# arotem3/CuDDHelmholtz

Hardware: AMD Instinct MI355X
Metric: DDH-GMRES DoF*iter/s (higher is better)
Workload: dtype f32

## Files before the change

### cuddhelmholtz_amd/_native.py

```python
from __future__ import annotations

import ctypes as C
import re
from pathlib import Path

ROOT = Path(__file__).resolve().parent.parent
LIB_PATH = Path(__file__).resolve().parent / "lib" / "libcuddh_amd.so"
HEADERS = [ROOT / "include" / "cuddh_hip.h", ROOT / "include" / "cuddh_capi.h"]


class NativeLibraryMissing(RuntimeError):
    pass


def declared_symbols() -> list[str]:
    names: list[str] = []
    for h in HEADERS:
        text = re.sub(r"/\*.*?\*/", "", h.read_text(), flags=re.S)
        for m in re.finditer(r"\b(cuddh_[a-z0-9_]+)\s*\(", text):
            n = m.group(1)
            if n not in names and n != "cuddh_action_cb":
                names.append(n)
    return names

# ... 138 lines not shown
_sig("cuddh_hip_operator_plan_apply", ci, vp, cd, ci, vp, vp, vp)
_sig("cuddh_hip_ddh_geom_setup_f32", ci, ci, ci, ci, ci, vp, vp, vp, vp, vp, vp)
_sig("cuddh_hip_ddh_geom_setup_f64", ci, ci, ci, ci, ci, vp, vp, vp, vp, vp, vp)
_sig("cuddh_hip_ddh_geom_from_corners_f32", ci, ci, ci, vp, vp, vp, vp, vp, vp, vp)
_sig("cuddh_hip_ddh_geom_from_corners_f64", ci, ci, ci, vp, vp, vp, vp, vp, vp, vp)
_sig("cuddh_hip_ddh_plan_create", ci, C.POINTER(vp), C.POINTER(DdhDesc), ci, ci)
_sig("cuddh_hip_ddh_plan_create_general", ci, C.POINTER(vp), C.POINTER(DdhDesc), ci, ci, ci)
_sig("cuddh_hip_ddh_plan_destroy", ci, vp)
_sig("cuddh_hip_ddh_plan_kernel", ci, vp)
_sig("cuddh_hip_ddh_plan_set_wh_iters", ci, vp, ci)
_sig("cuddh_hip_ddh_plan_set_wave_priority", ci, vp, ci)
_sig("cuddh_hip_ddh_plan_set_sweep_form", ci, vp, ci)
_sig("cuddh_hip_ddh_plan_sweep_form", ci, vp)
_sig("cuddh_hip_ddh_plan_set_chain_order", ci, vp, ci)
_sig("cuddh_hip_ddh_plan_chain_order", ci, vp)
_sig("cuddh_hip_ddh_plan_set_owner_rule", ci, vp, ci)
_sig("cuddh_element_lane_tables", ci, ci, vp, vp, vp)
_sig("cuddh_ddh_resolve", ci, *([ci] * 13), vp)
_sig("cuddh_hip_ddh_plan_set_time_grids", ci, vp, ci, vp, vp, vp, vp, vp, vp)
_sig("cuddh_hip_ddh_plan_time_grids", ci, vp)
_sig("cuddh_hip_ddh_plan_set_integrator", ci, vp, ci)
_sig("cuddh_hip_ddh_plan_integrator", ci, vp)
_sig("cuddh_hip_ddh_apply_list_f32", ci, vp, vp, ci, vp, vp, ci, vp, vp, vp)
_sig("cuddh_hip_ddh_apply_list_f64", ci, vp, vp, ci, vp, vp, ci, vp, vp, vp)
_sig("cuddh_hip_ddh_plan_set_vector_layout", ci, vp, vp, ci)
_sig("cuddh_hip_ddh_apply_f32", ci, vp, ci, ci, vp, vp, ci, vp, vp, vp)
_sig("cuddh_hip_ddh_apply_f64", ci, vp, ci, ci, vp, vp, ci, vp, vp, vp)
_sig("cuddh_hip_wave_stage_begin_f64", ci, ci, cd, vp, vp, vp, vp, vp, vp, vp)
_sig("cuddh_hip_wave_stage_rk2_a_f64", ci, ci, cd, cd, cd, *([vp] * 10))
_sig("cuddh_hip_wave_stage_rk2_b_f64", ci, ci, cd, cd, cd, cd, *([vp] * 11))
for _n in ("1", "2", "3"):
    _sig(f"cuddh_hip_wave_stage_rk4_{_n}_f64", ci, ci, cd, cd, cd, *([vp] * 12))
_sig("cuddh_hip_wave_stage_rk4_4_f64", ci, ci, cd, cd, cd, cd, *([vp] * 13))
# ... 103 lines not shown
_sig("cuddh_ddh_create_labels", vp, cd, vp, vp, ci, vp, ci, ci)
_sig("cuddh_ddh_create_labels_integrator", vp, cd, vp, vp, ci, vp, ci, ci, ci, vp, ci, ci, ci)
_sig("cuddh_ddh_create_timegrid", vp, cd, vp, vp, ci, ci, ci, ci, ci, ci, vp, ci)
_sig("cuddh_ddh_time_ratios", ci, vp, vp)
_sig("cuddh_ddh_create_integrator", vp, cd, vp, vp, ci, ci, ci, ci, ci, ci, vp, ci, ci, ci)
_sig("cuddh_ddh_integrator", ci, vp, vp, vp)
_sig("cuddh_ddh_destroy", None, vp)
_sig("cuddh_ddh_size", ci, vp)
_sig("cuddh_ddh_info", ci, vp, vp, vp)
_sig("cuddh_ddh_set_wh_iters", ci, vp, ci)
_sig("cuddh_ddh_set_wave_priority", ci, vp, ci)
_sig("cuddh_ddh_set_sweep_form", ci, vp, ci)
_sig("cuddh_ddh_sweep_form", ci, vp)
_sig("cuddh_ddh_set_chain_order", ci, vp, ci)
_sig("cuddh_ddh_chain_order", ci, vp)
_sig("cuddh_ddh_set_owner_rule", ci, vp, ci)


class MultiGpuResult(C.Structure):
    _fields_ = [("success", ci), ("num_iter", ci), ("num_matvec", ci), ("n_res", ci), ("world", ci), ("used_rccl", ci),
                ("t_setup", cd), ("t_rhs", cd), ("t_gmres", cd), ("t_postprocess", cd), ("bytes_sent_per_action_rank0", C.c_longlong)]


class HelmholtzMultiGpuResult(C.Structure):
    _fields_ = [("success", ci), ("num_iter", ci), ("num_matvec", ci), ("n_res", ci), ("world", ci), ("used_rccl", ci),
                ("t_setup", cd), ("t_apply", cd), ("t_gmres", cd), ("n_loc_max", C.c_longlong), ("n_halo_max", C.c_longlong),
                ("halo_bytes_per_apply_max", C.c_longlong)]


_sig("cuddh_helmholtz_multi_gpu", ci, vp, ci, cd, vp, vp, vp, vp, ci, ci, ci, ci, ci, cd, C.POINTER(HelmholtzMultiGpuResult), vp)
# ... 62 lines not shown
```

### cuddhelmholtz_amd/api.py

```python
from __future__ import annotations

import ctypes as C
from dataclasses import dataclass, field

import numpy as np

from . import _native as N

lib = N.lib


def _ptr(t, dtype=None, numel=None, what="tensor"):
    if t is None:
        return None
    if not t.is_cuda:
        raise ValueError(f"{what}: expected a CUDA tensor")
    if not t.is_contiguous():
        raise ValueError(f"{what}: expected a contiguous tensor")
    if dtype is not None:
        import torch

        want = {"f64": torch.float64, "f32": torch.float32, "i32": torch.int32}.get(dtype, dtype)
        if t.dtype != want:
            raise ValueError(f"{what}: expected dtype {want}, got {t.dtype}")
# ... 504 lines not shown
    def sweep_form(self) -> int:
        form = lib.cuddh_ddh_sweep_form(self._h)
        if form < 0:
            N.check_capi(form, "DDH.sweep_form")
        return form

    def set_chain_order(self, order: int = 0):
        N.check_capi(lib.cuddh_ddh_set_chain_order(self._h, int(order)), "DDH.set_chain_order")

    def chain_order(self) -> int:
        order = lib.cuddh_ddh_chain_order(self._h)
        if order < 0:
            N.check_capi(order, "DDH.chain_order")
        return order

    def set_owner_rule(self, last: bool):
        N.check_capi(lib.cuddh_ddh_set_owner_rule(self._h, 1 if last else 0), "DDH.set_owner_rule")

    def set_wave_priority(self, high: bool):
        N.check_capi(lib.cuddh_ddh_set_wave_priority(self._h, 1 if high else 0), "DDH.set_wave_priority")

    def table(self, name: str) -> np.ndarray:
        n = lib.cuddh_ddh_table(self._h, name.encode(), None, 1)
        if n < 0:
            raise RuntimeError(N.last_error())
        dtype = np.int32 if name in self._INT_TABLES else (np.float64 if self.f64 else np.float32)
        out = np.empty(int(n), dtype=dtype)
        if n:
            lib.cuddh_ddh_table(self._h, name.encode(), _h(out), 0)
        return out
# ... 288 lines not shown
```

### cuddhelmholtz_amd/csrc/include/cuddh/ddh.hpp

```cpp
#ifndef CUDDH_AMD_DDH_HPP
#define CUDDH_AMD_DDH_HPP

#include <memory>
#include <vector>

#include "blas1.hpp"
#include "ensemble.hpp"
#include "krylov.hpp"
#include "memory.hpp"
#include "operator.hpp"
#include "operators.hpp"

struct cuddh_ddh_plan;

namespace cuddh
{
    struct from_labels_t
    {
        explicit constexpr from_labels_t() = default;
    };
    inline constexpr from_labels_t from_labels{};

    struct DDHTimeStep
    {
// ... 47 lines not shown
            int num_domains() const { return n_domains; }
            int num_steps() const { return nt; }
            double time_step() const { return dt; }
            int mesh_steps() const;
            DDHIntegrator integrator() const;
            const std::vector<int> &time_ratios() const;
            const std::vector<int> &time_grid_ratios() const;
            long long time_grid_table(int ratio, int which, const Real *&table) const;
            int kernel_kind() const;
            void set_waveholtz_iterations(int n) const;
            void set_wave_priority(bool high) const;
            void set_sweep_form(int form) const;
            int sweep_form() const;
            void set_chain_order(int order) const;
            int chain_order() const;
            void set_last_copy_publishes(bool last) const;
            const EnsembleSpace &ensemble() const { return *efem; }

            void solve(int dom_begin, int dom_end, const double *x, double *y, bool zero_y, const Real *lambda,
                       Real *update) const;
            void solve_listed(const int *d_domains, int n, const double *x, const Real *lambda, Real *update) const;
            void solve_listed(const int *d_domains, int n, const double *x, double *y, bool zero_y, const Real *lambda, Real *update) const;

            const host_device_ivec &table_B() const { return _Bf; }
            const host_device_ivec &table_gI() const { return _gI; }
            const host_device_ivec &table_sI() const { return _sI; }
            const HostDeviceArray<Real> &table_D() const { return _D; }
            const HostDeviceArray<Real> &table_G() const
            {
                ensure_plan();
// ... 103 lines not shown
```

### cuddhelmholtz_amd/csrc/kernels/ddh.hip

```cpp
#include <algorithm>
#include <cmath>
#include <type_traits>
#include <vector>

#include "ddh_device.hpp"
#include "ddh_element_lane.hpp"
#include "ddh_resolve.hpp"
#include "element_lane_tables.hpp"

using namespace cuddh_k;

struct cuddh_ddh_plan;

namespace
{
    template <typename Real>
    using DdhRun = void (*)(const cuddh_ddh_plan *, const DdhArgs<Real> &, int n_local, hipStream_t);
    struct DdhLaunch
    {
        DdhRun<float> run32 = nullptr;
        DdhRun<double> run64 = nullptr;
        int per_group = 4;
        unsigned block = 256;
        size_t lds = 0;
// ... 7 lines not shown
    DdhResolved now{0, 0, 0};
    DdhLaunch launch;
    unsigned facts = 0;
    int mx_elems = 0;
    int nodes;
    int wh_iters = 5;
    const int *gI_override = nullptr;
    int g_ndof_override = 0;
    float *Aop = nullptr;
    double *Aop64 = nullptr;
    float *Sep = nullptr;
    float *Sep4 = nullptr;
    int last_copy = 0;
    int sweep_form = 0;
    int chain_order = 0;
    int wave_priority = 0;
    int *csr_off = nullptr, *csr_src = nullptr;
    int requested = 0;
    int n_grids = 0;
    void *grids = nullptr;
    const int *grid_of = nullptr;
    const void *grid_filter = nullptr, *grid_cs = nullptr, *grid_sn = nullptr;
    int *by_steps = nullptr;
    int *by_index = nullptr;
    int rk4 = 0;
};

namespace
{
    constexpr int WH_ITERS_REFERENCE = 5;
// ... 1456 lines not shown
                                        { hipLaunchKernelGGL((ddh_wave8_kernel<Real, ASM, SEP>), launch_grid(p, n_local), dim3(p->launch.block), 0, st, A,
                                                             static_cast<const Real *>(p->d.D), fl, cs, sn, reinterpret_cast<const Real *>(p->Sep)); });
    }

    template <typename Real, bool GRIDS, bool RK4>
    void run_mfma(const cuddh_ddh_plan *p, const DdhArgs<Real> &A, int n_local, hipStream_t st)
    {
        const Real *K = sizeof(Real) == 4 ? reinterpret_cast<const Real *>(p->Aop) : reinterpret_cast<const Real *>(p->Aop64);
        with_tables<Real, GRIDS, RK4>(p, [&](const Real *fl, const Real *cs, const Real *sn, auto... o)
                                      { with_flags([&](auto FORCED, auto HOLD)
                                                   { hipLaunchKernelGGL((ddh_mfma_kernel<Real, FORCED.value, HOLD.value, decltype(o)...>), launch_grid(p, n_local),
                                                                        dim3(p->launch.block), 0, st, A, K, fl, cs, sn, o...); },
                                                   A.x != nullptr, A.prio != 0); });
    }

    template <int NB, bool LAST_COPY, bool PAIRED, bool GRIDS>
    void run_element_lane(const cuddh_ddh_plan *p, const DdhArgs<float> &A, int n_local, hipStream_t st)
    {
        with_tables<float, GRIDS, false>(p, [&](const float *fl, const float *cs, const float *sn, auto... o)
                                         { with_flags([&](auto FORCED, auto HOLD)
                                                      { hipLaunchKernelGGL((ddh_element_lane_kernel<NB, FORCED.value, HOLD.value, LAST_COPY, PAIRED, decltype(o)...>),
                                                                           launch_grid(p, n_local), dim3(p->launch.block), 0, st, A, p->Sep4, fl, cs, sn, o...); },
                                                      A.x != nullptr, A.prio != 0); });
    }

    template <bool LAST_COPY, bool GRIDS>
    void run_element_lane8(const cuddh_ddh_plan *p, const DdhArgs<float> &A, int n_local, hipStream_t st)
    {
        with_tables<float, GRIDS, false>(p, [&](const float *fl, const float *cs, const float *sn, auto... o)
                                         { with_flags([&](auto FORCED, auto HOLD)
                                                      { hipLaunchKernelGGL((ddh_element_lane8_kernel<FORCED.value, HOLD.value, LAST_COPY, decltype(o)...>),
                                                                           launch_grid(p, n_local), dim3(p->launch.block), 0, st, A, p->Sep4, fl, cs, sn, o...); },
                                                      A.x != nullptr, A.prio != 0); });
    }

    template <typename Real, bool GRIDS, bool RK4>
    void set_launch(const cuddh_ddh_plan *p, const DdhResolved &r, DdhLaunch &L)
    {
        constexpr bool f32 = sizeof(Real) == 4, plain = !GRIDS && !RK4;
        DdhRun<Real> run = nullptr;
        const bool last_copy = p->last_copy != 0;
        switch (r.kernel)
        {
        case 1:
        case 10:
            L.per_group = 1;
            L.block = p->nodes;
            L.lds = (size_t)p->nodes * (4 * sizeof(Real) + 5 * sizeof(int));
            with_n_basis(p->d.nb, [&](auto NB)
                         {
                             if (p->nodes <= 256)
                                 run = r.kernel == 10 ? run_block<Real, NB.value, true, 256, GRIDS, RK4> : run_block<Real, NB.value, false, 256, GRIDS, RK4>;
// ... 6 lines not shown
            if constexpr (!RK4)
                run = run_wave<Real, f32 ? 1 : 0, GRIDS, RK4>;
            break;
        case 4:
            if constexpr (!RK4)
                run = run_wave<Real, f32 ? 2 : 0, GRIDS, RK4>;
            break;
        case 5:
            if constexpr (f32)
            {
                if (r.form < 2)
                    run = run_mfma<float, GRIDS, RK4>;
                else if constexpr (plain)
                {
                    L.per_group = 16;
                    with_flags([&](auto LAST_COPY, auto PAIRED) { run = run_element_lane<4, LAST_COPY.value, PAIRED.value, false>; }, r.form == 3, r.order == 2);
                }
            }
            break;
        case 8:
            if constexpr (!f32)
                run = run_mfma<double, GRIDS, RK4>;
            break;
        case 6:
        case 7:
            if constexpr (plain)
            {
                L.per_group = 8;
                if constexpr (f32)
                    run = r.kernel == 7 ? run_wave8<float, true, true> : run_wave8<float, true, false>;
                else if (r.kernel == 6)
                    run = run_wave8<double, false, false>;
            }
            break;
        case 9: run = run_general_wave<Real, f32 ? 1 : 0, GRIDS, RK4>; break;
        case 11:
            if constexpr (f32 && !RK4)
                with_flags([&](auto LAST_COPY) { run = run_element_lane8<LAST_COPY.value, GRIDS>; }, last_copy);
            break;
        case 12:
            if constexpr (f32 && plain)
            {
                L.per_group = 16;
                with_flags([&](auto LAST_COPY) { run = run_element_lane<5, LAST_COPY.value, false, false>; }, last_copy);
            }
            break;
        case 13:
            if constexpr (f32 && !RK4)
            {
                L.per_group = 16;
                with_flags(
                    [&](auto LAST_COPY)
                    {
                        if (p->d.nb == 4)
                            run = run_element_lane<4, LAST_COPY.value, false, GRIDS>;
                        else
                            run = run_element_lane<5, LAST_COPY.value, false, GRIDS>;
                    },
                    last_copy);
            }
            break;
        }
        if constexpr (f32)
            L.run32 = run;
        else
            L.run64 = run;
    }

    int resolve(cuddh_ddh_plan *p, int setting = DDH_SET_NONE)
    {
        const DdhShape shape{p->d.nb, p->d.nel1d, p->d.n_domains, p->is_f64, p->mx_elems};
        DdhResolved r;
        if (ddh_resolve(shape, p->requested, p->facts, p->now.kernel, DdhOptions{p->n_grids > 0, p->rk4, p->sweep_form, p->chain_order}, setting, r))
            return static_cast<int>(hipErrorInvalidValue);
        DdhLaunch L;
        with_flags([&](auto F64, auto GRIDS, auto RK4) { set_launch<std::conditional_t<F64.value, double, float>, GRIDS.value, RK4.value>(p, r, L); },
                   p->is_f64 != 0, p->n_grids > 0, p->rk4 != 0);
        if (!L.run32 && !L.run64)
            return static_cast<int>(hipErrorInvalidValue);
        p->now = r;
        p->launch = L;
        return 0;
    }

    template <class Store>
    int set_and_resolve(cuddh_ddh_plan *p, int setting, Store store)
    {
        const cuddh_ddh_plan before = *p;
        store(*p);
        const int err = resolve(p, setting);
        if (err)
            *p = before;
        return err;
    }

// ... 250 lines not shown
            return static_cast<int>(hipErrorInvalidValue);
        return set_and_resolve(plan, DDH_SET_SWEEP_FORM, [&](cuddh_ddh_plan &p) { p.sweep_form = form; });
    }

    int cuddh_hip_ddh_plan_sweep_form(const cuddh_ddh_plan *plan) { return plan ? plan->now.form : 0; }

    int cuddh_hip_ddh_plan_set_chain_order(cuddh_ddh_plan *plan, int order)
    {
        if (!plan)
            return static_cast<int>(hipErrorInvalidValue);
        return set_and_resolve(plan, DDH_SET_CHAIN_ORDER, [&](cuddh_ddh_plan &p) { p.chain_order = order; });
    }

    int cuddh_hip_ddh_plan_chain_order(const cuddh_ddh_plan *plan) { return plan ? plan->now.order : 0; }

    int cuddh_hip_ddh_plan_set_time_grids(cuddh_ddh_plan *plan, int n_grids, const int *h_nt, const double *h_dt, const void *filter,
                                          const void *cs, const void *sn, const int *d_grid_of)
    {
        if (!plan || n_grids < 1 || !h_nt || !h_dt || !filter || !cs || !sn || !d_grid_of)
            return static_cast<int>(hipErrorInvalidValue);
        const int nd = plan->d.n_domains;
        std::vector<int> filt_off(n_grids), cs_off(n_grids);
        long long fo = 0, co = 0;
        for (int g = 0; g < n_grids; ++g)
        {
            if (h_nt[g] < 1 || !(h_dt[g] > 0.0) || !std::isfinite(h_dt[g]))
                return static_cast<int>(hipErrorInvalidValue);
            filt_off[g] = static_cast<int>(fo);
            cs_off[g] = static_cast<int>(co);
            fo += (long long)h_nt[g] + 1;
// ... 117 lines not shown
```

### cuddhelmholtz_amd/csrc/kernels/ddh_element_lane.hpp

```cpp
#ifndef CUDDH_AMD_DDH_ELEMENT_LANE_HPP
#define CUDDH_AMD_DDH_ELEMENT_LANE_HPP

#include <type_traits>

#include "ddh_device.hpp"

namespace
{
#define CUDDH_EL_ASSEMBLE(NAME, SHL, SHR)                                                                                                  \
    __device__ inline void NAME(float (&hi)[4], float (&lo)[4], float mHi, float mLo)                                                      \
    {                                                                                                                                      \
        float t0, t1, t2, t3;                                                                                                              \
        asm volatile("s_nop 1\n\t"                                                                                                         \
                     "v_mul_f32_dpp %8, %0, %13 " SHR " row_mask:0xf bank_mask:0xf bound_ctrl:1\n\t"                                       \
                     "v_mul_f32_dpp %9, %1, %13 " SHR " row_mask:0xf bank_mask:0xf bound_ctrl:1\n\t"                                       \
                     "v_mul_f32_dpp %10, %2, %13 " SHR " row_mask:0xf bank_mask:0xf bound_ctrl:1\n\t"                                      \
                     "v_mul_f32_dpp %11, %3, %13 " SHR " row_mask:0xf bank_mask:0xf bound_ctrl:1\n\t"                                      \
                     "v_fmac_f32_dpp %0, %4, %12 " SHL " row_mask:0xf bank_mask:0xf bound_ctrl:1\n\t"                                      \
                     "v_fmac_f32_dpp %1, %5, %12 " SHL " row_mask:0xf bank_mask:0xf bound_ctrl:1\n\t"                                      \
                     "v_fmac_f32_dpp %2, %6, %12 " SHL " row_mask:0xf bank_mask:0xf bound_ctrl:1\n\t"                                      \
                     "v_fmac_f32_dpp %3, %7, %12 " SHL " row_mask:0xf bank_mask:0xf bound_ctrl:1\n\t"                                      \
                     "v_add_f32 %4, %4, %8\n\t"                                                                                            \
                     "v_add_f32 %5, %5, %9\n\t"                                                                                            \
                     "v_add_f32 %6, %6, %10\n\t"                                                                                           \
// ... 113 lines not shown
    {
        constexpr int EX = NEL - 1, EY = NEL * (NEL - 1);
        const int k = n % NB, l = n / NB;
        const bool first = !(k == 0 && (tid & EX) > 0) && !(l == 0 && (tid & EY) > 0);
        const bool last = !(k == NB - 1 && (tid & EX) < EX) && !(l == NB - 1 && (tid & EY) < EY);
        return LAST_COPY ? last : first;
    }

    typedef float pair_t __attribute__((ext_vector_type(2)));
    constexpr int el_pair(int k, int l) { return k + 4 * ((l == 1 || l == 2) ? 1 : 0); }
    constexpr int el_half(int l) { return l >= 2 ? 1 : 0; }
    constexpr unsigned ELEMENT_INTERIOR_PAIRS = (1u << 5) | (1u << 6);
    constexpr unsigned ELEMENT_LANE_DM_PAIRS(bool forced) { return forced ? 0x60u : 0x1fu; }
    constexpr unsigned ELEMENT_LANE_PAIRED_DM_PAIRS(bool forced) { return forced ? 0x60u : 0xffu; }

    __device__ inline pair_t pk_fma(pair_t a, pair_t b, pair_t c) { return __builtin_elementwise_fma(a, b, c); }
    __device__ inline pair_t pk_fma(float a, pair_t b, pair_t c) { return __builtin_elementwise_fma(pair_t{a, a}, b, c); }
    template <int HALF>
    __device__ inline void pk_fmac_scalar(pair_t &t, pair_t c, pair_t w)
    {
        if constexpr (HALF == 0)
            asm("v_pk_fma_f32 %0, %1, %2, %0 op_sel_hi:[0,1,1]" : "+v"(t) : "s"(c), "v"(w));
        else
            asm("v_pk_fma_f32 %0, %1, %2, %0 op_sel:[1,0,0] op_sel_hi:[1,1,1]" : "+v"(t) : "s"(c), "v"(w));
    }
    constexpr int bx_slot(int k, int j) { return 3 * k + (j < k ? j : j - 1); }
    template <int HALF>
    __device__ inline void pk_fmac_half(pair_t &t, pair_t c, pair_t w)
    {
        if constexpr (HALF == 0)
// ... 160 lines not shown
                    if (((INTERIOR >> l) & 1u) != 0)
                        dq = LEAN == 2 ? pk_fma(s1, Gf[l], pk_fma(c1, F[l], z[l])) : z[l];
                    else
                        dq = pk_fma(s1, Gf[l], pk_fma(c1, F[l], pk_fma(-Hi[l], qh[l], z[l])));
                    if (((DM >> l) & 1u) != 0)
                        q[l] = pk_fma(dm[l], dq, q[l]);
                    else
                        q[l] = pk_fma(hm[l], 2.0f * dq, q[l]);
                    u[l] = pk_fma(kw, p[l], u[l]);
                    v[l] = pk_fma(kw, q[l], v[l]);
                }
            }
        }
    }


    template <int NB, bool FORCED, bool HOLD, bool LAST_COPY, bool PAIRED, typename... Grids>
    __global__ void __launch_bounds__(256, NB == 4 ? 3 : (FORCED ? 1 : 2))
        ddh_element_lane_kernel(DdhArgs<float> A, const float *__restrict__ Sep, const float *__restrict__ filt, const float *__restrict__ cs,
                                const float *__restrict__ sn, Grids... grids)
    {
        constexpr bool GROUPED = sizeof...(Grids) > 0;
        constexpr int NN = NB * NB;
        constexpr int NS = NB == 4 ? 8 : NN;
        using state_t = std::conditional_t<NB == 4, pair_t, float>;
        static_assert(NB == 4 || NB == 5, "the assembly statements exist for 4 and 5 values a side");
        static_assert(sizeof...(Grids) <= 1 && scheme_of<Grids...> == 0, "one grid, or TimeGrids; no RK4 form");
        static_assert(!(PAIRED && NB != 4), "the paired chains are those of the packed form");
        static_assert(!(PAIRED && sizeof...(Grids) > 0), "the paired chains are built for the one-grid kernel only");
        const int s_first = A.dom_begin + 4 * (blockIdx.x * 4 + (threadIdx.x >> 6));
        if (s_first >= A.dom_end)
            return;
        if constexpr (HOLD)
            __builtin_amdgcn_s_setprio(3);
        [[maybe_unused]] const int w_first = wave_uniform(s_first);
        [[maybe_unused]] int done = 0;
        [[maybe_unused]] GroupedRows rows{};
        [[maybe_unused]] DdhArgs<float> Ap;
        const DdhArgs<float> &Ar = [&]() -> const DdhArgs<float> &
        {
            if constexpr (GROUPED)
                return Ap;
            else
                return A;
// ... 94 lines not shown
                for (int l = 0; l < 5; ++l)
                {
                    z[4 + 5 * l] = hi[l];
                    z[0 + 5 * l] = lo[l];
                }
                float up[5] = {z[20], z[21], z[22], z[23], z[24]}, dn[5] = {z[0], z[1], z[2], z[3], z[4]};
                element_assemble_eta_row5_asm(up, dn);
#pragma unroll
                for (int k = 0; k < 5; ++k)
                {
                    z[k + 20] = up[k];
                    z[k] = dn[k];
                }
            }
        };
        if constexpr (NB == 4)
            wh_march_pairs<FORCED ? 2 : 1, ELEMENT_INTERIOR_PAIRS, PAIRED ? ELEMENT_LANE_PAIRED_DM_PAIRS(FORCED) : ELEMENT_LANE_DM_PAIRS(FORCED)>(
                Ar, tg.nt, tg.dt, tg.filt, tg.cs, tg.sn, invm, Hi, F, Gf, u, v, sweep);
        else
            wh_march<FORCED ? 2 : 1, element_interior_registers(NB)>(Ar, tg.nt, tg.dt, tg.filt, tg.cs, tg.sn, invm, Hi, F, Gf, u, v, sweep);

        if constexpr (GROUPED)
        {
            tid = lane_here();
            asm volatile("" : "+s"(done));
            reread_args(Ap);
        }
        else
        {
            tid = threadIdx.x;
            asm volatile("" : "+v"(tid));
// ... 102 lines not shown
```

### cuddhelmholtz_amd/csrc/kernels/ddh_resolve.hpp

```cpp
#pragma once

namespace cuddh_k
{
    enum DdhCheck
    {
        DDH_STRUCTURE = 1,
        DDH_UNIFORM = 2,
        DDH_INTERIOR = 3,
        DDH_DENSE = 4,
        DDH_SEP8 = 5,
        DDH_LANE = 6
    };
    constexpr unsigned ddh_fact(int check) { return 1u << check; }

    struct DdhShape
    {
        int nb, nel1d, n_domains, is_f64;
        int mx_elems;
    };

    struct DdhOptions
    {
        int time_grids;
        int rk4;
        int sweep_form, chain_order;
    };

    enum DdhSetting
    {
        DDH_SET_NONE = 0,
        DDH_SET_SWEEP_FORM = 1,
        DDH_SET_CHAIN_ORDER = 2,
        DDH_SET_OWNER_RULE = 3
    };

    struct DdhResolved
    {
        int kernel;
        int form;
        int order;
    };

    constexpr int DDH_BLOCK_MAX_NODES = 1024;
    constexpr int DDH_GENERAL_MAX_NODES = 256;

    int ddh_checks(const DdhShape &shape, int request);

    int ddh_resolve(const DdhShape &shape, int request, unsigned facts, int current, const DdhOptions &options, int setting, DdhResolved &out);
}
```

### cuddhelmholtz_amd/csrc/src/capi.cpp

```cpp
#include <algorithm>
#include <cmath>
#include <cstdio>
#include <cstring>
#include <exception>
#include <memory>
#include <stdexcept>
#include <string>
#include <vector>

#include "cuddh.hpp"
#include "cuddh_capi.h"
#include "cuddh_hip.h"

using namespace cuddh;

namespace
{
    thread_local std::string g_error;

    template <typename F>
    int guarded(F &&f)
    {
        try
        {
// ... 1070 lines not shown
                h->f64->internals().set_chain_order(order);
            else
                h->f32->internals().set_chain_order(order);
        });
    }
    int cuddh_ddh_chain_order(void *d)
    {
        int order = 0;
        const int err = guarded([&]
        {
            auto *h = static_cast<DdhHandle *>(d);
            order = h->is64() ? h->f64->internals().chain_order() : h->f32->internals().chain_order();
        });
        return err ? -1 : order;
    }
    int cuddh_ddh_set_owner_rule(void *d, int last)
    {
        return guarded([&]
        {
            auto *h = static_cast<DdhHandle *>(d);
            if (h->is64())
                h->f64->internals().set_last_copy_publishes(last != 0);
            else
                h->f32->internals().set_last_copy_publishes(last != 0);
        });
    }
    int cuddh_ddh_sweep_form(void *d)
    {
        int form = 0;
        const int err = guarded([&]
// ... 392 lines not shown
```

### cuddhelmholtz_amd/csrc/src/ddh.cpp

```cpp
#include "cuddh/ddh.hpp"

#include <algorithm>
#include <atomic>
#include <chrono>
#include <cstdio>
#include <cstdlib>
#include <cmath>
#include <string>
#include <type_traits>
#include <vector>

#include "cuddh/parallel.hpp"
#include "cuddh/time_grid.hpp"
#include "cuddh_hip.h"

namespace cuddh
{
    namespace detail
    {
        namespace
        {
            template <typename Real>
            void geom_setup(int n_domains, int mx_elems, int nb, const int *n_elems, const int *elems, const double *w,
                            const double *points, const double *corners, Real *G)
// ... 653 lines not shown
        template <typename Real>
        void DDHCore<Real>::set_chain_order(int order) const
        {
            ensure_plan();
            check_hip(cuddh_hip_ddh_plan_set_chain_order(plan, order), "DDH chain order");
        }

        template <typename Real>
        int DDHCore<Real>::chain_order() const
        {
            ensure_plan();
            return cuddh_hip_ddh_plan_chain_order(plan);
        }

        template <typename Real>
        void DDHCore<Real>::set_last_copy_publishes(bool last) const
        {
            ensure_plan();
            check_hip(cuddh_hip_ddh_plan_set_owner_rule(plan, last ? 1 : 0), "DDH owner rule");
        }

        template <typename Real>
        void DDHCore<Real>::set_wave_priority(bool high) const
        {
            ensure_plan();
            check_hip(cuddh_hip_ddh_plan_set_wave_priority(plan, high ? 1 : 0), "DDH wave priority");
        }

        template <typename Real>
        void DDHCore<Real>::ensure_assembly() const
// ... 223 lines not shown
```

### cuddhelmholtz_amd/csrc/src/ddh_resolve.cpp

```cpp
#include "ddh_resolve.hpp"

#include "cuddh_hip.h"

namespace cuddh_k
{
    namespace
    {
        constexpr int REFUSED = 1;

        constexpr int ELEMENT_LANE_MIN_DOMAINS = 8192;
        constexpr int ELEMENT_LANE5_MIN_DOMAINS = 64;

        constexpr unsigned S = DDH_STRUCTURE, U = DDH_UNIFORM, I = DDH_INTERIOR;
        constexpr unsigned seq(unsigned a, unsigned b = 0, unsigned c = 0, unsigned d = 0, unsigned e = 0)
        {
            return a | (b << 4) | (c << 8) | (d << 12) | (e << 16);
        }

        struct KernelTraits
        {
            int nb, nel1d;
            int real_bytes;
            unsigned checks;
            bool grids, rk4, owner_rule;
// ... 109 lines not shown
                return REFUSED;
            k = k == 3 ? 2 : 1;
        }
        const bool lane_form = k == 5 && (facts & ddh_fact(DDH_LANE)) && !o.time_grids && !o.rk4;
        if (o.sweep_form >= 2 && !lane_form)
            return REFUSED;
        if (setting == DDH_SET_CHAIN_ORDER && o.chain_order == 2 && !lane_form)
            return REFUSED;
        if (setting == DDH_SET_OWNER_RULE && !KERNELS[k].owner_rule)
            return REFUSED;
        out.kernel = k;
        out.form = k != 5 ? 0 : !lane_form ? 1 : o.sweep_form != 0 ? o.sweep_form : s.n_domains >= ELEMENT_LANE_MIN_DOMAINS ? 2 : 1;
        out.order = out.form < 2 ? 0 : o.chain_order != 0 ? o.chain_order : o.sweep_form == 0 ? 2 : 1;
        return 0;
    }
}

extern "C"
{
    int cuddh_ddh_resolve(int nb, int nel1d, int n_domains, int is_f64, int mx_elems, int request, int facts, int current, int time_grids, int rk4,
                          int sweep_form, int chain_order, int setting, int *out)
    {
        using namespace cuddh_k;
        if (!out)
            return 1;
        const DdhShape s{nb, nel1d, n_domains, is_f64 ? 1 : 0, mx_elems};
        out[3] = ddh_checks(s, request);
        DdhResolved r{0, 0, 0};
        const int err = ddh_resolve(s, request, static_cast<unsigned>(facts), current, DdhOptions{time_grids, rk4, sweep_form, chain_order}, setting, r);
        out[0] = r.kernel;
        out[1] = r.form;
        out[2] = r.order;
        return err;
    }
}
```

### include/cuddh_capi.h

```cpp
#ifndef CUDDH_CAPI_H
#define CUDDH_CAPI_H

#include <stddef.h>

#ifdef __cplusplus
extern "C" {
#endif

const char *cuddh_last_error(void);
void cuddh_set_stream(void *stream);
void *cuddh_get_stream(void);

int cuddh_quadrature(int n, int type, double *h_x, double *h_w);
void *cuddh_basis_create(int n);
void cuddh_basis_destroy(void *basis);
int cuddh_basis_eval(void *basis, int m, const double *h_x, double *h_P);
int cuddh_basis_deriv(void *basis, int m, const double *h_x, double *h_D);

void *cuddh_mesh_uniform_rect(int nx, double ax, double bx, int ny, double ay, double by);
void *cuddh_mesh_from_vertices(int n_pts, const double *h_xy, int n_elem, const int *h_elems);
void *cuddh_mesh_load(const char *dir);
void *cuddh_mesh_refined(void *mesh, int times);
int cuddh_mesh_partition(void *mesh, int n_parts, int *h_labels);
void cuddh_mesh_destroy(void *mesh);
// ... 80 lines not shown
    double t_setup, t_apply, t_gmres;
    long long n_loc_max, n_halo_max, halo_bytes_per_apply_max;
} cuddh_helmholtz_multi_gpu_result;
int cuddh_helmholtz_multi_gpu(void *mesh, int nb, double omega, const double *h_a2x, const double *h_ax, const double *h_x, double *h_y,
                              int world, int transport, int reps, int m, int maxit, double tol, cuddh_helmholtz_multi_gpu_result *out,
                              double *h_res );
int cuddh_helmholtz_partition_query(void *mesh, void *fem, void *fs, int rank, int world, int which, int peer, int *h_out);
int cuddh_trace_exchange_query(const int *h_B, int n_domains, int mx_fdof, int n_lambda, int rank, int world, int which, int peer,
                               int *h_out);
int cuddh_ddh_set_wh_iters(void *ddh, int n);
int cuddh_ddh_set_wave_priority(void *ddh, int high);
int cuddh_ddh_set_sweep_form(void *ddh, int form);
int cuddh_ddh_sweep_form(void *ddh);
int cuddh_ddh_set_chain_order(void *ddh, int order);
int cuddh_ddh_chain_order(void *ddh);
int cuddh_ddh_set_owner_rule(void *ddh, int last);
int cuddh_ddh_rhs(void *ddh, const double *f, void *b);
int cuddh_ddh_postprocess(void *ddh, const void *lambda, const double *f, double *u);
int cuddh_ddh_action(void *ddh, const void *x, void *y);
int cuddh_ddh_local_traces(void *ddh, int d0, int d1, const double *f, const void *lambda, void *update);
int cuddh_ddh_local_traces_listed(void *ddh, const int *d_domains, int n, const double *f, const void *lambda, void *update);
int cuddh_ddh_local_solution_listed(void *ddh, const int *d_domains, int n, const void *lambda, const double *f, double *u, int zero_u);
int cuddh_ddh_local_solution(void *ddh, int d0, int d1, const void *lambda, const double *f, double *u, int zero_u);
long long cuddh_ddh_table(void *ddh, const char *name, void *h_out, int count_only);

typedef struct cuddh_solver_result
{
    int success;
    int num_iter;
    int num_matvec;
// ... 67 lines not shown
```

### include/cuddh_hip.h

```cpp
#ifndef CUDDH_HIP_H
#define CUDDH_HIP_H

#include <stddef.h>

#ifdef __cplusplus
extern "C" {
#endif


int cuddh_hip_malloc_zeroed(void **ptr, size_t bytes);
int cuddh_hip_free(void *ptr);
int cuddh_hip_copy_h2d(void *dst, const void *h_src, size_t bytes);
int cuddh_hip_copy_d2h(void *h_dst, const void *src, size_t bytes);
int cuddh_hip_copy_h2d_on(void *dst, const void *h_src, size_t bytes, void *stream);
int cuddh_hip_copy_d2h_on(void *h_dst, const void *src, size_t bytes, void *stream);
int cuddh_hip_copy_d2d(void *dst, const void *src, size_t bytes, void *stream);
int cuddh_hip_memset_zero(void *ptr, size_t bytes, void *stream);
int cuddh_hip_stream_sync(void *stream);
int cuddh_hip_device_sync(void);
int cuddh_hip_device_count(void);
int cuddh_hip_host_alloc(void **ptr, size_t bytes);
int cuddh_hip_host_free(void *ptr);
int cuddh_hip_copy_d2h_async(void *h_dst, const void *src, size_t bytes, void *stream);
int cuddh_hip_event_create(void **ev);
// ... 141 lines not shown
    const void *sn;
} cuddh_ddh_desc;

typedef struct cuddh_ddh_plan cuddh_ddh_plan;
int cuddh_hip_ddh_plan_create(cuddh_ddh_plan **plan, const cuddh_ddh_desc *desc, int is_f64, int kernel);
int cuddh_hip_ddh_plan_create_general(cuddh_ddh_plan **plan, const cuddh_ddh_desc *desc, int mx_elems, int is_f64, int kernel);
int cuddh_hip_ddh_plan_destroy(cuddh_ddh_plan *plan);
int cuddh_hip_ddh_plan_kernel(const cuddh_ddh_plan *plan);
int cuddh_hip_ddh_plan_set_vector_layout(cuddh_ddh_plan *plan, const int *d_gI, int g_ndof);
int cuddh_hip_ddh_plan_set_wave_priority(cuddh_ddh_plan *plan, int high);
int cuddh_hip_ddh_plan_set_wh_iters(cuddh_ddh_plan *plan, int wh_iters);
int cuddh_hip_ddh_plan_set_sweep_form(cuddh_ddh_plan *plan, int form);
int cuddh_hip_ddh_plan_sweep_form(const cuddh_ddh_plan *plan);
int cuddh_hip_ddh_plan_set_chain_order(cuddh_ddh_plan *plan, int order);
int cuddh_hip_ddh_plan_chain_order(const cuddh_ddh_plan *plan);
int cuddh_hip_ddh_plan_set_owner_rule(cuddh_ddh_plan *plan, int last);
int cuddh_element_lane_tables(int nb, const float *h_D, const float *h_G, float *h_out);
int cuddh_ddh_resolve(int nb, int nel1d, int n_domains, int is_f64, int mx_elems, int request, int facts, int current, int time_grids, int rk4,
                      int sweep_form, int chain_order, int setting, int *out);
int cuddh_hip_ddh_plan_set_time_grids(cuddh_ddh_plan *plan, int n_grids, const int *h_nt, const double *h_dt, const void *filter,
                                      const void *cs, const void *sn, const int *d_grid_of);
int cuddh_hip_ddh_plan_time_grids(const cuddh_ddh_plan *plan);
int cuddh_hip_ddh_plan_set_integrator(cuddh_ddh_plan *plan, int scheme);
int cuddh_hip_ddh_plan_integrator(const cuddh_ddh_plan *plan);

int cuddh_hip_ddh_apply_f32(const cuddh_ddh_plan *plan, int dom_begin, int dom_end, const double *x, double *y,
                            int zero_y, const float *lambda, float *update, void *stream);
int cuddh_hip_ddh_apply_f64(const cuddh_ddh_plan *plan, int dom_begin, int dom_end, const double *x, double *y,
                            int zero_y, const double *lambda, double *update, void *stream);
int cuddh_hip_ddh_apply_list_f32(const cuddh_ddh_plan *plan, const int *d_domains, int n, const double *x, double *y, int zero_y,
                                 const float *lambda, float *update, void *stream);
int cuddh_hip_ddh_apply_list_f64(const cuddh_ddh_plan *plan, const int *d_domains, int n, const double *x, double *y, int zero_y,
                                 const double *lambda, double *update, void *stream);

// ... 106 lines not shown
```

Baseline: 118.1 million.

## Apply wave-march sources only in first WH pass and reuse forced response

Adds a packed wave-march variant for the paired-chain element-lane kernel. The source terms are applied only in the first WaveHoltz pass. That forced response is parked in shared memory and added back after each later pass, which runs source-free, relying on linearity. The variant is selected by a new forcing setting that defaults to on when the chain order resolves to paired. This removes the per-step source FMAs and cos/sin table loads from later passes. In exchange it adds a large shared-memory buffer that may lower occupancy, and it changes the floating-point summation order.

```diff
diff --git a/cuddhelmholtz_amd/_native.py b/cuddhelmholtz_amd/_native.py
--- a/cuddhelmholtz_amd/_native.py
+++ b/cuddhelmholtz_amd/_native.py
@@ -176,9 +176,12 @@
 _sig("cuddh_hip_ddh_plan_sweep_form", ci, vp)
 _sig("cuddh_hip_ddh_plan_set_chain_order", ci, vp, ci)
 _sig("cuddh_hip_ddh_plan_chain_order", ci, vp)
+_sig("cuddh_hip_ddh_plan_set_forcing", ci, vp, ci)
+_sig("cuddh_hip_ddh_plan_forcing", ci, vp)
 _sig("cuddh_hip_ddh_plan_set_owner_rule", ci, vp, ci)
 _sig("cuddh_element_lane_tables", ci, ci, vp, vp, vp)
 _sig("cuddh_ddh_resolve", ci, *([ci] * 13), vp)
+_sig("cuddh_ddh_resolve_forcing", ci, *([ci] * 14), vp)
 _sig("cuddh_hip_ddh_plan_set_time_grids", ci, vp, ci, vp, vp, vp, vp, vp, vp)
 _sig("cuddh_hip_ddh_plan_time_grids", ci, vp)
 _sig("cuddh_hip_ddh_plan_set_integrator", ci, vp, ci)
@@ -312,6 +315,8 @@
 _sig("cuddh_ddh_sweep_form", ci, vp)
 _sig("cuddh_ddh_set_chain_order", ci, vp, ci)
 _sig("cuddh_ddh_chain_order", ci, vp)
+_sig("cuddh_ddh_set_forcing", ci, vp, ci)
+_sig("cuddh_ddh_forcing", ci, vp)
 _sig("cuddh_ddh_set_owner_rule", ci, vp, ci)
 
 
diff --git a/cuddhelmholtz_amd/api.py b/cuddhelmholtz_amd/api.py
--- a/cuddhelmholtz_amd/api.py
+++ b/cuddhelmholtz_amd/api.py
@@ -542,6 +542,15 @@
             N.check_capi(order, "DDH.chain_order")
         return order
 
+    def set_forcing(self, forcing: int = 0):
+        N.check_capi(lib.cuddh_ddh_set_forcing(self._h, int(forcing)), "DDH.set_forcing")
+
+    def forcing(self) -> int:
+        forcing = lib.cuddh_ddh_forcing(self._h)
+        if forcing < 0:
+            N.check_capi(forcing, "DDH.forcing")
+        return forcing
+
     def set_owner_rule(self, last: bool):
         N.check_capi(lib.cuddh_ddh_set_owner_rule(self._h, 1 if last else 0), "DDH.set_owner_rule")
 
diff --git a/cuddhelmholtz_amd/csrc/include/cuddh/ddh.hpp b/cuddhelmholtz_amd/csrc/include/cuddh/ddh.hpp
--- a/cuddhelmholtz_amd/csrc/include/cuddh/ddh.hpp
+++ b/cuddhelmholtz_amd/csrc/include/cuddh/ddh.hpp
@@ -85,6 +85,8 @@
             int sweep_form() const;
             void set_chain_order(int order) const;
             int chain_order() const;
+            void set_forcing(int forcing) const;
+            int forcing() const;
             void set_last_copy_publishes(bool last) const;
             const EnsembleSpace &ensemble() const { return *efem; }
 
diff --git a/cuddhelmholtz_amd/csrc/kernels/ddh.hip b/cuddhelmholtz_amd/csrc/kernels/ddh.hip
--- a/cuddhelmholtz_amd/csrc/kernels/ddh.hip
+++ b/cuddhelmholtz_amd/csrc/kernels/ddh.hip
@@ -45,6 +45,8 @@
     int last_copy = 0;
     int sweep_form = 0;
     int chain_order = 0;
+    int forcing = 0;
+    int forcing_now = 0;
     int wave_priority = 0;
     int *csr_off = nullptr, *csr_src = nullptr;
     int requested = 0;
@@ -1531,12 +1533,12 @@
                                                    A.x != nullptr, A.prio != 0); });
     }
 
-    template <int NB, bool LAST_COPY, bool PAIRED, bool GRIDS>
+    template <int NB, bool LAST_COPY, bool PAIRED, bool ONCE, bool GRIDS>
     void run_element_lane(const cuddh_ddh_plan *p, const DdhArgs<float> &A, int n_local, hipStream_t st)
     {
         with_tables<float, GRIDS, false>(p, [&](const float *fl, const float *cs, const float *sn, auto... o)
                                          { with_flags([&](auto FORCED, auto HOLD)
-                                                      { hipLaunchKernelGGL((ddh_element_lane_kernel<NB, FORCED.value, HOLD.value, LAST_COPY, PAIRED, decltype(o)...>),
+                                                      { hipLaunchKernelGGL((ddh_element_lane_kernel<NB, FORCED.value, HOLD.value, LAST_COPY, PAIRED, ONCE, decltype(o)...>),
                                                                            launch_grid(p, n_local), dim3(p->launch.block), 0, st, A, p->Sep4, fl, cs, sn, o...); },
                                                       A.x != nullptr, A.prio != 0); });
     }
@@ -1552,7 +1554,7 @@
     }
 
     template <typename Real, bool GRIDS, bool RK4>
-    void set_launch(const cuddh_ddh_plan *p, const DdhResolved &r, DdhLaunch &L)
+    void set_launch(const cuddh_ddh_plan *p, const DdhResolved &r, int forcing, DdhLaunch &L)
     {
         constexpr bool f32 = sizeof(Real) == 4, plain = !GRIDS && !RK4;
         DdhRun<Real> run = nullptr;
@@ -1589,7 +1591,9 @@
                 else if constexpr (plain)
                 {
                     L.per_group = 16;
-                    with_flags([&](auto LAST_COPY, auto PAIRED) { run = run_element_lane<4, LAST_COPY.value, PAIRED.value, false>; }, r.form == 3, r.order == 2);
+                    with_flags([&](auto LAST_COPY, auto PAIRED, auto ONCE)
+                               { run = run_element_lane<4, LAST_COPY.value, PAIRED.value, PAIRED.value && ONCE.value, false>; },
+                               r.form == 3, r.order == 2, forcing == 2);
                 }
             }
             break;
@@ -1617,7 +1621,7 @@
             if constexpr (f32 && plain)
             {
                 L.per_group = 16;
-                with_flags([&](auto LAST_COPY) { run = run_element_lane<5, LAST_COPY.value, false, false>; }, last_copy);
+                with_flags([&](auto LAST_COPY) { run = run_element_lane<5, LAST_COPY.value, false, false, false>; }, last_copy);
             }
             break;
         case 13:
@@ -1628,9 +1632,9 @@
                     [&](auto LAST_COPY)
                     {
                         if (p->d.nb == 4)
-                            run = run_element_lane<4, LAST_COPY.value, false, GRIDS>;
+                            run = run_element_lane<4, LAST_COPY.value, false, false, GRIDS>;
                         else
-                            run = run_element_lane<5, LAST_COPY.value, false, GRIDS>;
+                            run = run_element_lane<5, LAST_COPY.value, false, false, GRIDS>;
                     },
                     last_copy);
             }
@@ -1648,12 +1652,17 @@
         DdhResolved r;
         if (ddh_resolve(shape, p->requested, p->facts, p->now.kernel, DdhOptions{p->n_grids > 0, p->rk4, p->sweep_form, p->chain_order}, setting, r))
             return static_cast<int>(hipErrorInvalidValue);
+        if (setting == DDH_SET_FORCING && ddh_forcing_accepted(shape, p->requested, p->facts, p->now.kernel,
+                                                               DdhOptions{p->n_grids > 0, p->rk4, p->sweep_form, p->chain_order}, p->forcing))
+            return static_cast<int>(hipErrorInvalidValue);
+        const int forcing = ddh_forcing(r, p->sweep_form, p->chain_order, p->forcing);
         DdhLaunch L;
-        with_flags([&](auto F64, auto GRIDS, auto RK4) { set_launch<std::conditional_t<F64.value, double, float>, GRIDS.value, RK4.value>(p, r, L); },
+        with_flags([&](auto F64, auto GRIDS, auto RK4) { set_launch<std::conditional_t<F64.value, double, float>, GRIDS.value, RK4.value>(p, r, forcing, L); },
                    p->is_f64 != 0, p->n_grids > 0, p->rk4 != 0);
         if (!L.run32 && !L.run64)
             return static_cast<int>(hipErrorInvalidValue);
         p->now = r;
+        p->forcing_now = forcing;
         p->launch = L;
         return 0;
     }
@@ -1934,6 +1943,15 @@
 
     int cuddh_hip_ddh_plan_chain_order(const cuddh_ddh_plan *plan) { return plan ? plan->now.order : 0; }
 
+    int cuddh_hip_ddh_plan_set_forcing(cuddh_ddh_plan *plan, int forcing)
+    {
+        if (!plan)
+            return static_cast<int>(hipErrorInvalidValue);
+        return set_and_resolve(plan, DDH_SET_FORCING, [&](cuddh_ddh_plan &p) { p.forcing = forcing; });
+    }
+
+    int cuddh_hip_ddh_plan_forcing(const cuddh_ddh_plan *plan) { return plan ? plan->forcing_now : 0; }
+
     int cuddh_hip_ddh_plan_set_time_grids(cuddh_ddh_plan *plan, int n_grids, const int *h_nt, const double *h_dt, const void *filter,
                                           const void *cs, const void *sn, const int *d_grid_of)
     {
diff --git a/cuddhelmholtz_amd/csrc/kernels/ddh_element_lane.hpp b/cuddhelmholtz_amd/csrc/kernels/ddh_element_lane.hpp
--- a/cuddhelmholtz_amd/csrc/kernels/ddh_element_lane.hpp
+++ b/cuddhelmholtz_amd/csrc/kernels/ddh_element_lane.hpp
@@ -151,6 +151,9 @@
     constexpr unsigned ELEMENT_LANE_DM_PAIRS(bool forced) { return forced ? 0x60u : 0x1fu; }
     constexpr unsigned ELEMENT_LANE_PAIRED_DM_PAIRS(bool forced) { return forced ? 0x60u : 0xffu; }
 
+    constexpr unsigned ELEMENT_LANE_ONCE_FIRST_DM_PAIRS(bool forced) { return forced ? 0x00u : 0xffu; }
+    constexpr unsigned ELEMENT_LANE_ONCE_DM_PAIRS = 0xffu;
+
     __device__ inline pair_t pk_fma(pair_t a, pair_t b, pair_t c) { return __builtin_elementwise_fma(a, b, c); }
     __device__ inline pair_t pk_fma(float a, pair_t b, pair_t c) { return __builtin_elementwise_fma(pair_t{a, a}, b, c); }
     template <int HALF>
@@ -341,8 +344,109 @@
         }
     }
 
-
-    template <int NB, bool FORCED, bool HOLD, bool LAST_COPY, bool PAIRED, typename... Grids>
+    template <int LEAN, unsigned INTERIOR, unsigned DM, unsigned DM2, int N, typename Sweep>
+    __device__ inline void wh_march_pairs_once(const DdhArgs<float> &A, const int nt, const float dt, const float *__restrict__ filt,
+                                               const float *__restrict__ cs, const float *__restrict__ sn, const pair_t (&invm)[N],
+                                               const pair_t (&Hi)[N], const pair_t (&F)[N], const pair_t (&Gf)[N], pair_t (&u)[N], pair_t (&v)[N],
+                                               Sweep sweep)
+    {
+        static_assert(LEAN == 1 || LEAN == 2, "the packed loop has wh_march's LEAN forms only");
+        __shared__ pair_t parked[2 * N][256];
+        pair_t p[N], q[N], hm[N];
+        const float half_dt = 0.5f * dt;
+#pragma unroll
+        for (int l = 0; l < N; ++l)
+        {
+            p[l] = q[l] = u[l] = v[l] = 0;
+            hm[l] = half_dt * invm[l];
+        }
+        auto pass = [&](auto SOURCES, auto MASK, const pair_t(&dm)[N])
+        {
+            const float k0 = filt[0];
+#pragma unroll
+            for (int l = 0; l < N; ++l)
+            {
+                p[l] = u[l];
+                q[l] = v[l];
+                u[l] *= k0;
+                v[l] *= k0;
+            }
+            for (int it = 1; it <= nt; ++it)
+            {
+                [[maybe_unused]] float c0, s0, c1, s1;
+                if constexpr (SOURCES.value)
+                {
+                    c0 = cs[2 * it - 2], s0 = sn[2 * it - 2];
+                    c1 = cs[2 * it - 1], s1 = sn[2 * it - 1];
+                }
+                const float kw = filt[it];
+                pair_t z[N], ph[N], qh[N];
+
+                sweep(p, z);
+#pragma unroll
+                for (int l = 0; l < N; ++l)
+                {
+                    pair_t dq = ((INTERIOR >> l) & 1u) != 0 ? z[l] : pk_fma(-Hi[l], q[l], z[l]);
+                    if constexpr (SOURCES.value)
+                        if (((INTERIOR >> l) & 1u) == 0 || LEAN == 2)
+                            dq = pk_fma(s0, Gf[l], pk_fma(c0, F[l], dq));
+                    ph[l] = pk_fma(-half_dt, q[l], p[l]);
+                    qh[l] = pk_fma(hm[l], dq, q[l]);
+                    p[l] = pk_fma(-dt, qh[l], p[l]);
+                }
+                sweep(ph, z);
+#pragma unroll
+                for (int l = 0; l < N; ++l)
+                {
+                    pair_t dq = ((INTERIOR >> l) & 1u) != 0 ? z[l] : pk_fma(-Hi[l], qh[l], z[l]);
+                    if constexpr (SOURCES.value)
+                        if (((INTERIOR >> l) & 1u) == 0 || LEAN == 2)
+                            dq = pk_fma(s1, Gf[l], pk_fma(c1, F[l], dq));
+                    if (((MASK.value >> l) & 1u) != 0)
+                        q[l] = pk_fma(dm[l], dq, q[l]);
+                    else
+                        q[l] = pk_fma(hm[l], 2.0f * dq, q[l]);
+                    u[l] = pk_fma(kw, p[l], u[l]);
+                    v[l] = pk_fma(kw, q[l], v[l]);
+                }
+            }
+        };
+        if (A.wh_iters < 1)
+            return;
+        pair_t(*const r)[256] = reinterpret_cast<pair_t(*)[256]>(&parked[0][threadIdx.x]);
+        {
+            pair_t dm[N];
+#pragma unroll
+            for (int l = 0; l < N; ++l)
+                dm[l] = ((DM >> l) & 1u) != 0 ? dt * invm[l] : pair_t{0.0f, 0.0f};
+            pass(std::true_type{}, std::integral_constant<unsigned, DM>{}, dm);
+        }
+        if (A.wh_iters < 2)
+            return;
+#pragma unroll
+        for (int l = 0; l < N; ++l)
+        {
+            r[l][0] = u[l];
+            r[N + l][0] = v[l];
+        }
+        pair_t dm2[N];
+#pragma unroll
+        for (int l = 0; l < N; ++l)
+            dm2[l] = ((DM2 >> l) & 1u) != 0 ? hm[l] + hm[l] : pair_t{0.0f, 0.0f};
+        for (int whit = 1; whit < A.wh_iters; ++whit)
+        {
+            pass(std::false_type{}, std::integral_constant<unsigned, DM2>{}, dm2);
+#pragma unroll
+            for (int l = 0; l < N; ++l)
+            {
+                u[l] += r[l][0];
+                v[l] += r[N + l][0];
+            }
+        }
+    }
+
+
+    template <int NB, bool FORCED, bool HOLD, bool LAST_COPY, bool PAIRED, bool ONCE, typename... Grids>
     __global__ void __launch_bounds__(256, NB == 4 ? 3 : (FORCED ? 1 : 2))
         ddh_element_lane_kernel(DdhArgs<float> A, const float *__restrict__ Sep, const float *__restrict__ filt, const float *__restrict__ cs,
                                 const float *__restrict__ sn, Grids... grids)
@@ -355,6 +459,7 @@
         static_assert(sizeof...(Grids) <= 1 && scheme_of<Grids...> == 0, "one grid, or TimeGrids; no RK4 form");
         static_assert(!(PAIRED && NB != 4), "the paired chains are those of the packed form");
         static_assert(!(PAIRED && sizeof...(Grids) > 0), "the paired chains are built for the one-grid kernel only");
+        static_assert(!(ONCE && !PAIRED), "the march with the sources in the first pass only is built beside the paired chains only");
         const int s_first = A.dom_begin + 4 * (blockIdx.x * 4 + (threadIdx.x >> 6));
         if (s_first >= A.dom_end)
             return;
@@ -479,7 +584,10 @@
                 }
             }
         };
-        if constexpr (NB == 4)
+        if constexpr (NB == 4 && ONCE)
+            wh_march_pairs_once<FORCED ? 2 : 1, ELEMENT_INTERIOR_PAIRS, ELEMENT_LANE_ONCE_FIRST_DM_PAIRS(FORCED), ELEMENT_LANE_ONCE_DM_PAIRS>(
+                Ar, tg.nt, tg.dt, tg.filt, tg.cs, tg.sn, invm, Hi, F, Gf, u, v, sweep);
+        else if constexpr (NB == 4)
             wh_march_pairs<FORCED ? 2 : 1, ELEMENT_INTERIOR_PAIRS, PAIRED ? ELEMENT_LANE_PAIRED_DM_PAIRS(FORCED) : ELEMENT_LANE_DM_PAIRS(FORCED)>(
                 Ar, tg.nt, tg.dt, tg.filt, tg.cs, tg.sn, invm, Hi, F, Gf, u, v, sweep);
         else
diff --git a/cuddhelmholtz_amd/csrc/kernels/ddh_resolve.hpp b/cuddhelmholtz_amd/csrc/kernels/ddh_resolve.hpp
--- a/cuddhelmholtz_amd/csrc/kernels/ddh_resolve.hpp
+++ b/cuddhelmholtz_amd/csrc/kernels/ddh_resolve.hpp
@@ -31,7 +31,8 @@
         DDH_SET_NONE = 0,
         DDH_SET_SWEEP_FORM = 1,
         DDH_SET_CHAIN_ORDER = 2,
-        DDH_SET_OWNER_RULE = 3
+        DDH_SET_OWNER_RULE = 3,
+        DDH_SET_FORCING = 4
     };
 
     struct DdhResolved
@@ -47,4 +48,8 @@
     int ddh_checks(const DdhShape &shape, int request);
 
     int ddh_resolve(const DdhShape &shape, int request, unsigned facts, int current, const DdhOptions &options, int setting, DdhResolved &out);
+
+    int ddh_forcing(const DdhResolved &resolved, int sweep_form, int chain_order, int forcing);
+
+    int ddh_forcing_accepted(const DdhShape &shape, int request, unsigned facts, int current, const DdhOptions &options, int forcing);
 }
diff --git a/cuddhelmholtz_amd/csrc/src/capi.cpp b/cuddhelmholtz_amd/csrc/src/capi.cpp
--- a/cuddhelmholtz_amd/csrc/src/capi.cpp
+++ b/cuddhelmholtz_amd/csrc/src/capi.cpp
@@ -1108,6 +1108,27 @@
         });
         return err ? -1 : order;
     }
+    int cuddh_ddh_set_forcing(void *d, int forcing)
+    {
+        return guarded([&]
+        {
+            auto *h = static_cast<DdhHandle *>(d);
+            if (h->is64())
+                h->f64->internals().set_forcing(forcing);
+            else
+                h->f32->internals().set_forcing(forcing);
+        });
+    }
+    int cuddh_ddh_forcing(void *d)
+    {
+        int forcing = 0;
+        const int err = guarded([&]
+        {
+            auto *h = static_cast<DdhHandle *>(d);
+            forcing = h->is64() ? h->f64->internals().forcing() : h->f32->internals().forcing();
+        });
+        return err ? -1 : forcing;
+    }
     int cuddh_ddh_set_owner_rule(void *d, int last)
     {
         return guarded([&]
diff --git a/cuddhelmholtz_amd/csrc/src/ddh.cpp b/cuddhelmholtz_amd/csrc/src/ddh.cpp
--- a/cuddhelmholtz_amd/csrc/src/ddh.cpp
+++ b/cuddhelmholtz_amd/csrc/src/ddh.cpp
@@ -691,6 +691,20 @@
         }
 
         template <typename Real>
+        void DDHCore<Real>::set_forcing(int forcing) const
+        {
+            ensure_plan();
+            check_hip(cuddh_hip_ddh_plan_set_forcing(plan, forcing), "DDH forcing");
+        }
+
+        template <typename Real>
+        int DDHCore<Real>::forcing() const
+        {
+            ensure_plan();
+            return cuddh_hip_ddh_plan_forcing(plan);
+        }
+
+        template <typename Real>
         void DDHCore<Real>::set_last_copy_publishes(bool last) const
         {
             ensure_plan();
diff --git a/cuddhelmholtz_amd/csrc/src/ddh_resolve.cpp b/cuddhelmholtz_amd/csrc/src/ddh_resolve.cpp
--- a/cuddhelmholtz_amd/csrc/src/ddh_resolve.cpp
+++ b/cuddhelmholtz_amd/csrc/src/ddh_resolve.cpp
@@ -147,6 +147,25 @@
         out.order = out.form < 2 ? 0 : o.chain_order != 0 ? o.chain_order : o.sweep_form == 0 ? 2 : 1;
         return 0;
     }
+
+    int ddh_forcing(const DdhResolved &r, int sweep_form, int chain_order, int forcing)
+    {
+        if (r.order != 2)
+            return 0;
+        if (forcing == 2)
+            return 2;
+        return forcing == 0 && sweep_form == 0 && chain_order == 0 ? 2 : 1;
+    }
+
+    int ddh_forcing_accepted(const DdhShape &s, int request, unsigned facts, int current, const DdhOptions &o, int forcing)
+    {
+        if (forcing < 0 || forcing > 2)
+            return REFUSED;
+        if (forcing != 2)
+            return 0;
+        DdhResolved unused;
+        return ddh_resolve(s, request, facts, current, DdhOptions{o.time_grids, o.rk4, o.sweep_form, 2}, DDH_SET_CHAIN_ORDER, unused);
+    }
 }
 
 extern "C"
@@ -166,4 +185,23 @@
         out[2] = r.order;
         return err;
     }
+
+    int cuddh_ddh_resolve_forcing(int nb, int nel1d, int n_domains, int is_f64, int mx_elems, int request, int facts, int current, int time_grids, int rk4,
+                                  int sweep_form, int chain_order, int forcing, int setting, int *out)
+    {
+        using namespace cuddh_k;
+        if (!out)
+            return 1;
+        const DdhShape s{nb, nel1d, n_domains, is_f64 ? 1 : 0, mx_elems};
+        const DdhOptions o{time_grids, rk4, sweep_form, chain_order};
+        DdhResolved r{0, 0, 0};
+        int err = ddh_resolve(s, request, static_cast<unsigned>(facts), current, o, setting, r);
+        if (!err && (forcing < 0 || forcing > 2 || (setting == DDH_SET_FORCING && ddh_forcing_accepted(s, request, static_cast<unsigned>(facts), current, o, forcing))))
+            err = 1;
+        out[0] = err ? 0 : r.kernel;
+        out[1] = err ? 0 : r.form;
+        out[2] = err ? 0 : r.order;
+        out[3] = err ? 0 : ddh_forcing(r, sweep_form, chain_order, forcing);
+        return err;
+    }
 }
diff --git a/include/cuddh_capi.h b/include/cuddh_capi.h
--- a/include/cuddh_capi.h
+++ b/include/cuddh_capi.h
@@ -118,6 +118,8 @@
 int cuddh_ddh_sweep_form(void *ddh);
 int cuddh_ddh_set_chain_order(void *ddh, int order);
 int cuddh_ddh_chain_order(void *ddh);
+int cuddh_ddh_set_forcing(void *ddh, int forcing);
+int cuddh_ddh_forcing(void *ddh);
 int cuddh_ddh_set_owner_rule(void *ddh, int last);
 int cuddh_ddh_rhs(void *ddh, const double *f, void *b);
 int cuddh_ddh_postprocess(void *ddh, const void *lambda, const double *f, double *u);
diff --git a/include/cuddh_hip.h b/include/cuddh_hip.h
--- a/include/cuddh_hip.h
+++ b/include/cuddh_hip.h
@@ -179,10 +179,14 @@
 int cuddh_hip_ddh_plan_sweep_form(const cuddh_ddh_plan *plan);
 int cuddh_hip_ddh_plan_set_chain_order(cuddh_ddh_plan *plan, int order);
 int cuddh_hip_ddh_plan_chain_order(const cuddh_ddh_plan *plan);
+int cuddh_hip_ddh_plan_set_forcing(cuddh_ddh_plan *plan, int forcing);
+int cuddh_hip_ddh_plan_forcing(const cuddh_ddh_plan *plan);
 int cuddh_hip_ddh_plan_set_owner_rule(cuddh_ddh_plan *plan, int last);
 int cuddh_element_lane_tables(int nb, const float *h_D, const float *h_G, float *h_out);
 int cuddh_ddh_resolve(int nb, int nel1d, int n_domains, int is_f64, int mx_elems, int request, int facts, int current, int time_grids, int rk4,
                       int sweep_form, int chain_order, int setting, int *out);
+int cuddh_ddh_resolve_forcing(int nb, int nel1d, int n_domains, int is_f64, int mx_elems, int request, int facts, int current, int time_grids,
+                              int rk4, int sweep_form, int chain_order, int forcing, int setting, int *out);
 int cuddh_hip_ddh_plan_set_time_grids(cuddh_ddh_plan *plan, int n_grids, const int *h_nt, const double *h_dt, const void *filter,
                                       const void *cs, const void *sn, const int *d_grid_of);
 int cuddh_hip_ddh_plan_time_grids(const cuddh_ddh_plan *plan);
```

New measurement: 127.6 million, median of 6. 1.08x the previous value.
